# chto/linna

Hardware: AMD Instinct MI355X
Metric: emulator log-likelihood evals/sec (higher is better)
Workload: dtype f32; 1 GPU; 33-D Gaussian, 4x512 MLP emulator (33->512x4->33), nwalkers=4096 batched log-likelihood per GPU (BASELINE configs[1]); nwalkers_per_gpu=4096, launch=direct launches, parallelism=walkers sharded, 1 rank(s), no data-path collective

## Files before the change

include/linna_hip.h:

```cpp
#ifndef LINNA_HIP_H
#define LINNA_HIP_H
#include <stddef.h>
#include <stdint.h>

#ifdef __cplusplus
extern "C" {
#endif

#define LINNA_ABI_VERSION 12

typedef struct linna_ctx linna_ctx_t;
typedef struct linna_net linna_net_t;
typedef struct linna_logprob linna_logprob_t;
typedef struct linna_graph linna_graph_t;

int linna_abi_version(void);
const char* linna_last_error(void);
#define LINNA_OK 0
#define LINNA_ERR_INVALID (-1)
#define LINNA_ERR_HIP (-2)
#define LINNA_ERR_UNSUPPORTED (-3)
#define LINNA_ERR_INTERNAL (-4)
int linna_debug_raise(int kind);
int linna_ctx_create(int device, linna_ctx_t** out);
// ... 118 lines not shown
    const int* log10_flag; const float* xmean; const float* xstd;
    linna_colmap_t outmap;
    const float* S; int lds;
    const float* Ssym;
    const float* w;
    const float* gscale;
    float temperature;
    const float* Sfac;
} linna_logprob_desc_t;

int linna_logprob_create(linna_ctx_t* ctx, linna_net_t* net, const linna_logprob_desc_t* desc,
                         linna_logprob_t** out);
int linna_logprob_destroy(linna_logprob_t* lp);
int linna_weights_changed(linna_ctx_t* ctx);
#define LINNA_PRECISION_FP32 0
#define LINNA_PRECISION_BF16 1
int linna_logprob_set_precision(linna_logprob_t* lp, int precision);
int linna_logprob_precision(const linna_logprob_t* lp, int* out);
int linna_logprob_set_grad_precision(linna_logprob_t* lp, int precision);
int linna_logprob_grad_precision(const linna_logprob_t* lp, int* out);
int linna_engine_rows(int rows);
int linna_dense_tri(int mode);
int linna_serve_plain(int on);
int linna_program_plain(const linna_layer_t* layers, int nlayers, int in_size, int rows, int dense_nout);
int linna_logprob_serve_plain(linna_logprob_t* lp, int B, int* out);
int linna_logprob_grad_launches(linna_logprob_t* lp, int B, int* out);
int linna_slice_fusion(int mask);
int linna_program_describe(const linna_layer_t* layers, int nlayers, int in_size, int rows, int dense_nout, char* buf,
                           size_t n);
int linna_program_describe_grad_bf16(const linna_layer_t* layers, int nlayers, int in_size, int rows, char* buf, size_t n);
size_t linna_logprob_ws_bytes(const linna_logprob_t* lp, int B, int with_grad);
int linna_logprob_eval(linna_logprob_t* lp, const float* Z, int ldz, int B, void* ws, float* lnP,
                       float* THETA, int ldt, void* stream);
int linna_logprob_eval_if(linna_logprob_t* lp, const float* Z, int ldz, int B, void* ws, float* lnP,
                          float* THETA, int ldt, const int* gate, void* stream);
int linna_logprob_eval_slice_points(linna_logprob_t* lp, const float* coords, int ldc, int ndim, const int* S_idx,
                                    int ns, const float* DIR, int ldd, const float* w, int nrep, float* lnP,
                                    const int* gate, void* stream);
int linna_logprob_grad(linna_logprob_t* lp, const float* Z, int ldz, int B, void* ws, float* lnP,
                       float* G, int ldg, void* stream);
int linna_logprob_grad_leapfrog(linna_logprob_t* lp, float* Q, int ldq, int B, void* ws, float* lnP, float* G, int ldg,
                                float* P, int ldp, const float* mass, float eps_kick, float eps_drift, void* stream);

typedef struct {
    uint32_t struct_size;
    int nout;
// ... 165 lines not shown
```

linna_amd/_lib.py:

```python
import ctypes as C
import os

import torch

_HERE = os.path.dirname(os.path.abspath(__file__))
LIB_PATH = os.environ.get("LINNA_LIB_PATH") or os.path.join(_HERE, "liblinna_hip.so")
ABI_VERSION = 12

c_float_p = C.c_void_p
c_int_p = C.c_void_p


class _Sized(C.Structure):

    def __init__(self, *a, **k):
        C.Structure.__init__(self, *a, **k)
        self.struct_size = C.sizeof(type(self))


def sized_array(cls, n):
    arr = (cls * n)()
    for i in range(n):
        arr[i].struct_size = C.sizeof(cls)
    return arr
# ... 82 lines not shown
    "linna_linear_bwd": (_I, [_V, _V, _I, _V, _I, _V, _I, _V, _I, _V, _I, _V, _I, _V, _I, _I, _I, _F, _V]),
    "linna_net_create": (_I, [_V, C.POINTER(Layer), _I, _I, _PV]),
    "linna_net_destroy": (_I, [_V]),
    "linna_net_prepare": (_I, [_V, _I, _I]),
    "linna_net_fwd_ws_bytes": (_SZ, [_V, _I]),
    "linna_net_bwd_ws_bytes": (_SZ, [_V, _I]),
    "linna_net_forward": (_I, [_V, _V, _I, _I, _V, _V, _I, C.POINTER(ColMap), _V]),
    "linna_net_backward": (_I, [_V, _V, _I, _I, _V, _V, _V, _I, _V, _I, _I, _V]),
    "linna_net_stream_state": (_I, [_V, _V, _V, _V]),
    "linna_prior_map_fwd": (_I, [_V, _V, _I, _I, _I, _V, _V, _V, _V, _V, _V, _V, _I, _V, _I, _V]),
    "linna_prior_map_bwd": (_I, [_V, _V, _I, _I, _I, _V, _V, _V, _V, _V, _V, _I, _V, _I, _V]),
    "linna_gauss_loglike_diag": (_I, [_V, _V, _I, _I, _I, _V, _V, _I, _I, _F, _V, _V]),
    "linna_gauss_loglike_dense": (_I, [_V, _V, _I, _I, _I, _V, _I, _V, _I, _I, _F, _V, _V, _V]),
    "linna_logprob_create": (_I, [_V, _V, C.POINTER(LogprobDesc), _PV]),
    "linna_logprob_destroy": (_I, [_V]),
    "linna_weights_changed": (_I, [_V]),
    "linna_logprob_set_precision": (_I, [_V, _I]),
    "linna_logprob_precision": (_I, [_V, _V]),
    "linna_logprob_set_grad_precision": (_I, [_V, _I]),
    "linna_logprob_grad_precision": (_I, [_V, _V]),
    "linna_engine_rows": (_I, [_I]),
    "linna_dense_tri": (_I, [_I]),
    "linna_serve_plain": (_I, [_I]),
    "linna_program_plain": (_I, [_V, _I, _I, _I, _I]),
    "linna_logprob_serve_plain": (_I, [_V, _I, _V]),
    "linna_logprob_grad_launches": (_I, [_V, _I, _V]),
    "linna_slice_fusion": (_I, [_I]),
    "linna_net_train_launches": (_I, [_V, _I]),
    "linna_net_set_train_precision": (_I, [_V, _I]),
    "linna_net_train_precision": (_I, [_V, _V]),
    "linna_program_describe": (_I, [_V, _I, _I, _I, _I, _V, C.c_size_t]),
    "linna_program_describe_grad_bf16": (_I, [_V, _I, _I, _I, _V, C.c_size_t]),
    "linna_logprob_ws_bytes": (_SZ, [_V, _I, _I]),
    "linna_logprob_eval": (_I, [_V, _V, _I, _I, _V, _V, _V, _I, _V]),
    "linna_logprob_grad": (_I, [_V, _V, _I, _I, _V, _V, _V, _I, _V]),
    "linna_logprob_grad_leapfrog": (_I, [_V, _V, _I, _I, _V, _V, _V, _I, _V, _I, _V, _F, _F, _V]),
    "linna_loss_scratch_bytes": (_SZ, [_I, _I]),
    "linna_chi2_md": (_I, [_V, C.POINTER(LossDesc), _V, _I, _I, _V, _V, _V]),
    "linna_chi2_ratio_loss_fwd_bwd": (_I, [_V, C.POINTER(LossDesc), _V, _I, _V, _I, _V, _V, _I, _V, _V, _V, _V, _I, _F, _V]),
    "linna_net_prepare_loss": (_I, [_V, C.POINTER(LossDesc)]),
    "linna_loss_targets": (_I, [_V, C.POINTER(LossDesc), _V, _I, _I, _V, _I, _V]),
    "linna_net_forward_loss": (_I, [_V, C.POINTER(LossDesc), _V, _I, _V, _I, _V, _V, _V, _V, _I, _V, _V, _I, _V, _I, _V, _F, _V, _V, _V, _I,
                                    _V, _V, _F, _F, _V]),
    "linna_net_train_step": (_I, [_V, C.POINTER(LossDesc), _V, _I, _V, _I, _V, _V, _V, _V, _I, _V, _V, _I, _V, _I, _V, _F, _V, _V, _V, _I,
                                  _V, _V, _V, _F, _F, _V]),
    "linna_net_train_step_update": (_I, [_V, C.POINTER(LossDesc), _V, _I, _V, _I, _V, _V, _V, _V, _I, _V, _V, _I, _V, _I, _V, _F, _V, _V, _V, _I,
# ... 168 lines not shown
class quiet_gc(object):

    def __enter__(self):
        import gc
        self.on = gc.isenabled() and os.environ.get("LINNA_QUIET_GC", "1") != "0"
        if self.on:
            gc.freeze()
        return self

    def __exit__(self, *exc):
        import gc
        if self.on:
            gc.unfreeze()
        return False


def slice_fusion(mask=-1):
    prev = load().linna_slice_fusion(int(mask))
    if prev < 0:
        check(prev)
    return prev


def serve_plain(on=-1):
    prev = load().linna_serve_plain(int(on))
    if prev < 0:
        check(prev)
    return prev


def engine_rows(rows=0):
    prev = load().linna_engine_rows(int(rows))
    if prev < 0:
        check(prev)
    return prev
```

linna_amd/csrc/api.hip:

```cpp
#include "common.h"

#include <stdarg.h>
#include <stdio.h>
#include <string.h>
#include <cstring>
#include <string>
#include <vector>
#include <atomic>
#include <new>
#include <stdlib.h>

namespace linna {

static thread_local std::string g_err;

void set_error(const char* fmt, ...) {
    char buf[512];
    va_list ap;
    va_start(ap, fmt);
    vsnprintf(buf, sizeof buf, fmt, ap);
    va_end(ap);
    g_err = buf;
}

// ... 1029 lines not shown
    if (!lp || !out) { set_error("logprob_grad_precision: null argument"); return LINNA_ERR_INVALID; }
    *out = lp->grad_precision;
    return LINNA_OK;
} LINNA_CATCH_INT
int linna_program_describe_grad_bf16(const linna_layer_t* layers, int nlayers, int in_size, int rows, char* buf, size_t n) try {
    if (!layers || nlayers < 1 || !buf || !n) { set_error("program_describe_grad_bf16: bad arguments"); return LINNA_ERR_INVALID; }
    TRY(check_layers(layers, nlayers, "program_describe_grad_bf16"));
    return net_stream_describe(NS_GRAD_INPUT_BF16, layers, nlayers, in_size, nullptr, rows, buf, n);
} LINNA_CATCH_INT
int linna_program_describe(const linna_layer_t* layers, int nlayers, int in_size, int rows, int dense_nout, char* buf, size_t n) try {
    if (!layers || nlayers < 1 || !buf || !n) { set_error("program_describe: bad arguments"); return LINNA_ERR_INVALID; }
    TRY(check_layers(layers, nlayers, "program_describe"));
    static float dummy;
    if (dense_nout == -1) return net_stream_describe(ns_grad_kind(layers, nlayers), layers, nlayers, in_size, nullptr, rows, buf, n);
    const int dn_cols = dense_nout < -1 ? -dense_nout : dense_nout;
    NsDense dn{&dummy, (dn_cols + 3) & ~3, nullptr, nullptr, dense_nout < -1 ? 1 : 0, net_stream_dense_tri(-1)};
    if (dn_cols > 0) return net_stream_describe(NS_SERVE_DENSE, layers, nlayers, in_size, &dn, rows, buf, n);
    return net_stream_describe(NS_SERVE, layers, nlayers, in_size, nullptr, rows, buf, n);
} LINNA_CATCH_INT
int linna_serve_plain(int on) try {
    if (on < -1 || on > 1) { set_error("linna_serve_plain: %d (-1 query, 0 or 1)", on); return LINNA_ERR_INVALID; }
    return net_stream_serve_plain(on);
} LINNA_CATCH_INT
int linna_program_plain(const linna_layer_t* layers, int nlayers, int in_size, int rows, int dense_nout) try {
    if (!layers || nlayers < 1) { set_error("program_plain: bad arguments"); return LINNA_ERR_INVALID; }
    TRY(check_layers(layers, nlayers, "program_plain"));
    if (dense_nout != 0) return 0;
    return net_stream_program_plain(NS_SERVE, layers, nlayers, in_size, nullptr, rows) ? 1 : 0;
} LINNA_CATCH_INT
int linna_logprob_serve_plain(linna_logprob_t* lp, int B, int* out) try {
    if (!lp || !out || B < 1) { set_error("logprob_serve_plain: bad arguments"); return LINNA_ERR_INVALID; }
    static float dummy[4];
    const LpRun r = lp_fused_run(lp, LpRun{dummy, 0, B, dummy}, dummy, LpLayout{});
    const NsDense dn = lp->dense();
    *out = !lp->bf16() && lp_serves_fused(lp, false) && !lp->dense_fused &&
           net_stream_takes_plain(lp->kind(), net_layers(lp->net, lp->kind()), lp_output(lp), r.lnP, r.D, r.TH, nullptr, nullptr, r.gate,
                                  net_stream_rows(B), lp->kind() == NS_SERVE_DENSE ? &dn : nullptr);
    return LINNA_OK;
} LINNA_CATCH_INT
int linna_dense_tri(int mode) try {
    if (mode < -1 || mode > 2) { set_error("linna_dense_tri: %d (-1 query, 0, 1 or 2)", mode); return LINNA_ERR_INVALID; }
    return net_stream_dense_tri(mode);
} LINNA_CATCH_INT
static std::atomic<int> g_slice_fusion{7};
static bool slice_derive_enabled() { return (g_slice_fusion.load() & 1) != 0; }
int linna_slice_fusion(int mode) try {
// ... 699 lines not shown
```

linna_amd/csrc/common.h:

```cpp
#pragma once
#include <hip/hip_runtime.h>
#include <stdint.h>
#include <exception>
#include "../../include/linna_hip.h"


typedef float f32x4 __attribute__((ext_vector_type(4)));
typedef float f32x16 __attribute__((ext_vector_type(16)));

namespace linna {

struct U4 { uint32_t x, y, z, w; };
__device__ __forceinline__ U4 philox4x32_10(U4 c, uint32_t k0, uint32_t k1) {
#pragma unroll
    for (int r = 0; r < 10; ++r) {
        const uint64_t p0 = (uint64_t)0xD2511F53u * c.x;
        const uint64_t p1 = (uint64_t)0xCD9E8D57u * c.z;
        U4 n;
        n.x = (uint32_t)(p1 >> 32) ^ c.y ^ k0;
        n.y = (uint32_t)p1;
        n.z = (uint32_t)(p0 >> 32) ^ c.w ^ k1;
        n.w = (uint32_t)p0;
        c = n;
        k0 += 0x9E3779B9u; k1 += 0xBB67AE85u;
// ... 265 lines not shown
    NS_SERVE_DENSE,
    NS_SERVE_BF16,
    NS_STORE,
    NS_TRAIN_FWD,
    NS_DX,
    NS_DX_INPUT,
    NS_GRAD_INPUT,
    NS_TRAIN_STEP,
    NS_TRAIN_STEP_BF16,
    NS_GRAD_INPUT_BF16,
    NS_GRAD_INPUT_WIDE,
};
inline bool ns_kind_full_layers(NsKind k) { return k == NS_SERVE || k == NS_SERVE_DENSE || k == NS_SERVE_BF16; }
struct NsPlan { bool ok; size_t packed_floats; bool grad_ok; const char* why; };
NsPlan net_stream_plan(NsKind kind, const linna_layer_t* layers, int nl, int in_size, const NsDense* dn = nullptr);
int net_stream_rows(int B);
int net_stream_force_rows(int rows);
inline NsKind ns_grad_kind(const linna_layer_t* layers, int nl) { return nl >= 1 && layers[nl - 1].N > 64 ? NS_GRAD_INPUT_WIDE : NS_GRAD_INPUT; }
bool net_stream_grad_fits(const linna_layer_t* layers, int nl, int in_size, int rows);
int launch_net_stream_pack(NsKind kind, const linna_layer_t* layers, int nl, int in_size, float* packed, int rows, const NsDense* dn,
                           hipStream_t s);
int net_stream_describe(NsKind kind, const linna_layer_t* layers, int nl, int in_size, const NsDense* dn, int rows, char* buf, size_t n);
int net_stream_serve_plain(int on);
bool net_stream_program_plain(NsKind kind, const linna_layer_t* layers, int nl, int in_size, const NsDense* dn, int rows);
bool net_stream_launch_plain_ok(bool cscale, bool cshift, bool w, bool cexp, bool lnP, bool D, bool TH, bool gate);
struct NsNet { const linna_layer_t* layers; int nl, in_size; };
struct NsInput { int nin; const int* is_flat; const float* a1; const float* a2; const int* lg; const float* xmean; const float* xstd; };
struct NsOutput { const float* cscale; const float* cshift; const float* cpost; const float* cshift2; const float* w; float T; };
struct NsOpBufs { float* y; int ldy; float* t; int ldt; const float* x; int ldx; const float* gate; float* dprev; int ldp; float* dt; int lddt; };
struct NsPost { const float* rows; int n; float scale; float* out; int* step; float* hyper; float b1, b2; };
int launch_net_stream_dx(const NsNet& net, const float* packed, const float* dOUT, int lddo, int B, const NsOpBufs* ops, int with_input,
                         int rows, hipStream_t s, const NsPost* post = nullptr);
struct NsMove {
    float* coords; int ldc; float* logp; const int* S;
    const float* cc; int ldcc; const int* C; int nc;
    unsigned long long seed; const int* step; int step_off; int stream; float a; int* naccept;
    int slice;
    float* chain = nullptr; float* lps = nullptr;
    const float* sl_Z0 = nullptr; const float* sl_L = nullptr; const float* sl_R = nullptr; const float* sl_Zt = nullptr;
    int sl_m = 0, sl_nt = 0; unsigned long long sl_seed = 0; const int* sl_step = nullptr; int sl_stream = 0;
    const int* sl_flags = nullptr;
    const SliceBegin* sb = nullptr;
};
int launch_net_stream_store(const NsNet& net, const float* packed, const float* X, int ldx, int B, const NsOpBufs* ops,
                            const float* cscale, const float* cshift, int rows, hipStream_t s);
struct NsTrainLoss { const float* YN; int ldyn;
// ... 82 lines not shown
```

linna_amd/csrc/net_program.hip:

```cpp
#include "net_program.h"
#include <stdlib.h>
#include <algorithm>
#include <atomic>
#include <cstring>
#include <mutex>
#include <string>
#include <unordered_map>

namespace linna {

size_t NsProgram::lds_for(int rows, bool grad) const {
    size_t b = (size_t)(2 * rows * LD + ((bias_total + 3) & ~3)) * sizeof(float) + 128 + (x0_keep ? 4096 : 0);
#ifdef NS_STAMPS
    b += NS_NW * 32 * 8;
#endif
    return b + (grad ? (size_t)mask_slots * 64 * NS_NW * sizeof(unsigned) : 0);
}

static int ceil16(int k) { return (k + 15) & ~15; }
int ns_seg_steps(const NsSeg& s) {
    if (s.type == NS_WIDE && s.zext < 0) return 2 * s.steps - 60;
    return s.type == NS_WIDE && s.zext > 0 ? s.steps + (s.passes - 1) * s.zext : s.steps * s.passes;
}
static int ns_switch(std::atomic<int>& sw, const char* name, int dflt, bool (*valid)(int)) {
// ... 376 lines not shown
    if (cache.size() >= 256) cache.clear();
    NsProgramRef p = std::make_shared<const NsProgram>(ns_build_kind(kind, layers, nl, in_size, dn, side));
    cache.emplace(std::move(key), p);
    return p;
}

bool ns_program_plain(const NsProgram& p) {
    if (!p.ok || p.bf || p.dense || p.x0_keep || p.side_f4 || p.nseg_f < 1) return false;
    for (int i = 0; i < p.nseg_f; ++i) {
        const NsSeg& g = p.seg[i];
        if (g.type != NS_WIDE && g.type != NS_SPLIT) return false;
        if (g.x0_col || (g.type == NS_WIDE && (g.zext || g.kslice))) return false;
    }
    return true;
}
bool net_stream_program_plain(NsKind kind, const linna_layer_t* layers, int nl, int in_size, const NsDense* dn, int rows) {
    return kind == NS_SERVE && rows == 16 && ns_program_plain(*ns_program(kind, layers, nl, in_size, dn, rows));
}
bool net_stream_launch_plain_ok(bool cscale, bool cshift, bool w, bool cexp, bool lnP, bool D, bool TH, bool gate) {
    return cscale && cshift && w && !cexp && lnP && !D && !TH && !gate;
}
static std::atomic<int> g_serve_plain{1};
int net_stream_serve_plain(int on) { return on < 0 ? g_serve_plain.load() : g_serve_plain.exchange(on ? 1 : 0); }

int ns_seg_cols(const NsProgram& p, const linna_layer_t* layers, int i) {
    const linna_layer_t& l = layers[p.seg_op[i]];
    return p.seg_hidden[i] ? l.C : i < p.nseg_f ? l.N : l.K;
}
NsGates ns_gates(const NsProgram& p, const linna_layer_t* layers, int nl, int rows) {
    NsGates g;
    for (int i = 0; i < NS_MAXSEG; ++i) g.gbit[i] = g.mbit[i] = -1;
    for (int i = 0; i < p.nseg_f; ++i) {
        const int op = p.seg_op[i];
        if (op >= nl || (!p.seg_hidden[i] && op == nl - 1)) continue;
        g.gbit[i] = g.ncols;
        g.ncols += (ns_seg_cols(p, layers, i) + 63) & ~63;
    }
    for (int i = p.nseg_f; i < (int)p.seg.size(); ++i) {
        const int op = p.seg_op[i];
        const bool hidden = p.seg_hidden[i] != 0;
        if (!hidden && !(op > 0 && (layers[op - 1].op == LINNA_OP_RESBLOCK || layers[op - 1].relu))) continue;
        const int src = hidden ? op : op - 1;
        for (int j = 0; j < p.nseg_f; ++j)
            if (p.seg_op[j] == src && (p.seg_hidden[j] != 0) == hidden) g.mbit[i] = g.gbit[j];
        if (g.mbit[i] < 0) g.ok = false;
    }
// ... 188 lines not shown
```

linna_amd/csrc/net_stream.hip:

```cpp
#include "net_program.h"
#include <stdlib.h>
#include <type_traits>
#include <cstring>
#include <algorithm>

namespace linna {

typedef __bf16 bf16x8 __attribute__((ext_vector_type(8)));
typedef short s16x4 __attribute__((ext_vector_type(4)));

#ifndef NS_R
#define NS_R 6
#endif
#ifndef NS_PRE
#define NS_PRE 2
#endif
struct NsArgs {
    const float* Z; int ldz; int B; int nin;
    const int* is_flat; const float* a1; const float* a2; const int* lg;
    const float* xmean; const float* xstd;
    const float* packed;
    int G, nseg, LD, kpad0, nout, bias_total;
    int Gstride, nseg_f;
    const float* gscale; float* Gout; int ldg;
// ... 159 lines not shown
template <int R, int MOVE, bool GRAD, int STORE, int ROWS, bool BF = false>
__global__ __launch_bounds__(64 * NS_NW, 1) void net_stream_kernel(NsArgs a) {
    constexpr bool EPS = false, PLAIN = false, WOUT = false;
#include "net_stream_body.inc"
}
template <int R, int MOVE, bool GRAD, int STORE, int ROWS, bool BF>
__global__ __launch_bounds__(64 * NS_NW, 1) void net_stream_eps_kernel(NsArgs a) {
    static_assert(!BF && GRAD && (STORE == 0 || STORE == 2) && MOVE == 0, "the fp32 one-launch gradients only");
    constexpr bool EPS = true, PLAIN = false, WOUT = false;
#include "net_stream_body.inc"
}
template <int R, int MOVE, bool GRAD, int STORE, int ROWS, bool BF, bool EPSV>
__global__ __launch_bounds__(64 * NS_NW, 1) void net_stream_wide_kernel(NsArgs a) {
    static_assert(!BF && GRAD && STORE == 2 && MOVE == 0, "the fp32 one-launch gradient of any network only");
    constexpr bool EPS = EPSV, PLAIN = false, WOUT = true;
#include "net_stream_body.inc"
}
template <int R>
__global__ __launch_bounds__(64 * NS_NW, 1) void net_stream_plain_kernel(NsArgs a) {
    constexpr int MOVE = 0, STORE = 0, ROWS = 16;
    constexpr bool GRAD = false, BF = false, EPS = false, PLAIN = true, WOUT = false;
#include "net_stream_body.inc"
}
template <int R, int MOVE, bool GRAD, int STORE, int ROWS, bool BF>
__global__ __launch_bounds__(64 * NS_NW, 1) void net_stream_train_bf16_kernel(NsArgs a) {
    static_assert(BF && GRAD && STORE == 3 && ROWS == 4 && MOVE == 0, "the bf16 training step only");
    constexpr bool EPS = false, PLAIN = false, WOUT = false;
#include "net_stream_body.inc"
}
template <int R, int MOVE, bool GRAD, int STORE, int ROWS, bool BF>
__global__ __launch_bounds__(64 * NS_NW, 1) void net_stream_slice_bf16_kernel(NsArgs a) {
    static_assert(BF && !GRAD && STORE == 0 && MOVE == 2, "the bf16 slice evaluation only");
    constexpr bool EPS = false, PLAIN = false, WOUT = false;
#define NS_BODY_SLICE_BF16
#include "net_stream_body.inc"
#undef NS_BODY_SLICE_BF16
}
template <int R, int MOVE, bool GRAD, int STORE, int ROWS, bool BF>
__global__ __launch_bounds__(64 * NS_NW, 1) void net_stream_grad_bf16_kernel(NsArgs a) {
    static_assert(BF && GRAD && STORE == 2 && MOVE == 0, "the bf16 one-launch gradient only");
    constexpr bool EPS = false, PLAIN = false, WOUT = false;
#define NS_BODY_GRAD_BF16
#include "net_stream_body.inc"
#undef NS_BODY_GRAD_BF16
}
template <int R, int MOVE, bool GRAD, int STORE, int ROWS, bool BF>
// ... 57 lines not shown
        if (rc != LINNA_OK) return rc;
        attr_set = true;
    }
    hipLaunchKernelGGL(Kernel, dim3(nblocks), dim3(64 * NS_NW), lds_bytes, s, a);
    return check_hip(hipGetLastError(), what);
}
template <int MOVE, bool GRAD, int STORE, int ROWS, bool BF = false, bool EPS = false>
static int ns_launch_rows(const NsArgs& a, int B, size_t lds_bytes, hipStream_t s, int extra = 0) {
    if constexpr (EPS) return ns_launch<net_stream_eps_kernel<NS_R, MOVE, GRAD, STORE, ROWS, BF>>(a, (B + ROWS - 1) / ROWS + extra, lds_bytes, s, "net_stream launch");
    else return ns_launch<net_stream_kernel<NS_R, MOVE, GRAD, STORE, ROWS, BF>>(a, (B + ROWS - 1) / ROWS + extra, lds_bytes, s, "net_stream launch");
}
template <int MOVE, bool GRAD, int STORE = 0, bool BF = false, bool EPS = false>
static int ns_launch_kernel(const NsArgs& a0, int B, const NsProgram& p, int rows, hipStream_t s, int extra = 0, size_t lds_extra = 0,
                            bool plain = false, bool wide = false) {
    const size_t lds = p.lds_for(rows, GRAD) + lds_extra;
#ifdef NS_STAMPS
    NsArgs a = a0;
    a.stamps = getenv("LINNA_FUSED_STAMPS") ? reinterpret_cast<unsigned long long*>(strtoull(getenv("LINNA_FUSED_STAMPS"), nullptr, 16)) : nullptr;
    if (!a.stamps) { set_error("net_stream: NS_STAMPS build needs LINNA_FUSED_STAMPS"); return LINNA_ERR_INVALID; }
#else
    const NsArgs& a = a0;
#endif
    if constexpr (MOVE == 0 && !GRAD && STORE == 0 && !BF && !EPS) {
        if (plain && rows == 16) return ns_launch<net_stream_plain_kernel<NS_R>>(a, (B + 15) / 16, lds, s, "net_stream plain launch");
    }
    if constexpr (MOVE == 0 && GRAD && STORE == 2 && !BF) {
        const char* const what = "net_stream wide-output gradient launch";
        if (wide && rows == 4) return ns_launch<net_stream_wide_kernel<NS_R, 0, true, 2, 4, false, EPS>>(a, (B + 3) / 4, lds, s, what);
        if (wide && rows == 8) return ns_launch<net_stream_wide_kernel<NS_R, 0, true, 2, 8, false, EPS>>(a, (B + 7) / 8, lds, s, what);
        if (wide && rows == 16) return ns_launch<net_stream_wide_kernel<NS_R, 0, true, 2, 16, false, EPS>>(a, (B + 15) / 16, lds, s, what);
    }
    if (rows == 4) return ns_launch_rows<MOVE, GRAD, STORE, 4, BF, EPS>(a, B, lds, s, extra);
    if constexpr (BF) {
        if (rows == 8) return ns_launch_rows<MOVE, GRAD, STORE, 8, BF, EPS>(a, B, lds, s, extra);
        if (rows == 16) return ns_launch_rows<MOVE, GRAD, STORE, 16, BF, EPS>(a, B, lds, s, extra);
    } else if constexpr (STORE == 3 && GRAD) {
    } else {
        if (rows == 8) return ns_launch_rows<MOVE, GRAD, STORE, 8, false, EPS>(a, B, lds, s, extra);
        if (rows == 16) return ns_launch_rows<MOVE, GRAD, STORE, 16, false, EPS>(a, B, lds, s, extra);
    }
    set_error("net_stream: %d rows per workgroup", rows);
    return LINNA_ERR_INVALID;
}
template <int ROWS>
static int ns_launch_slice_bf16_rows(const NsArgs& a, int B, size_t lds_bytes, hipStream_t s) {
    return ns_launch<net_stream_slice_bf16_kernel<NS_R, 2, false, 0, ROWS, true>>(a, (B + ROWS - 1) / ROWS, lds_bytes, s, "net_stream bf16 slice launch");
// ... 331 lines not shown
```

linna_amd/csrc/net_stream_body.inc:

```
    constexpr int NT = NS_NT, NW = NS_NW;
    constexpr int RG = 32;
    constexpr bool SM = ROWS < 16;
    constexpr int RS = SM ? ROWS / 4 : 1;
    constexpr int NQ = SM ? RS : NT;
    constexpr int NACC = SM ? 4 * RS : NT;
#ifdef NS_BODY_SLICE_BF16
    static_assert(BF && !GRAD && STORE == 0 && MOVE == 2, "bf16: the slice evaluation");
#elif defined(NS_BODY_GRAD_BF16)
    static_assert(BF && GRAD && STORE == 2 && MOVE == 0, "bf16: lnP and its gradient in one launch");
#else
    static_assert(!BF || (!GRAD && STORE == 0 && MOVE != 2) || (GRAD && STORE == 3 && MOVE == 0 && ROWS == 4),
                  "bf16: serving, the fused stretch move and the merged training step (4-row engine)");
#endif
    constexpr bool BFT = BF && GRAD && STORE == 3;
    constexpr int AK = BF ? 2 : 1;
    constexpr bool K4 = !SM && !BF && (STORE == 0 || (GRAD && STORE == 2));
    constexpr bool TRB = GRAD && STORE == 3;
    constexpr bool DXE = STORE == 2 || TRB;
    constexpr bool G2 = GRAD && STORE == 2;
    constexpr bool LB = G2;
    constexpr bool LATE_REFILL = true;
    constexpr bool RNAN = STORE == 1;
    auto relu_f = [](float v) { if constexpr (RNAN) return isnan(v) ? v : fmaxf(v, 0.f); else return fmaxf(v, 0.f); };
    static_assert(ROWS == 16 || ROWS == 8 || ROWS == 4, "rows per workgroup");
    static_assert(R % 2 == 0, "the A double buffer alternates with the ring slot parity");
    extern __shared__ __attribute__((aligned(16))) float smem[];
    const int LD = a.LD, ABUF = ROWS * LD;
    constexpr bool KA = STORE == 3 || STORE == 1 || GRAD;
    const NsArgs* const ka = KA ? reinterpret_cast<const NsArgs*>((const void*)__builtin_amdgcn_kernarg_segment_ptr()) : &a;
    float* const act = smem;
    float* const lbias = smem + 2 * ABUF;
    unsigned* const lbits = reinterpret_cast<unsigned*>(smem + a.bits_off);
    const int nbw = a.nbw;
    const int tid = threadIdx.x, lane = tid & 63;
    const int wave = __builtin_amdgcn_readfirstlane(tid >> 6);
    const int li = lane & 15, kq = lane >> 4;
    const int row0 = blockIdx.x * ROWS;
    if constexpr (!PLAIN) {
        if (a.gate && a.gate[0] == 0) return;
    }
    int mv_rows = a.B;
    if constexpr (MOVE == 2) {
        if (a.mv_C) {
            mv_rows = a.mv_step[0] * a.mv_step_off;
// ... 310 lines not shown
        if (j < nb4) reinterpret_cast<f32x4*>(lbias)[j] = breg[i];
    }
    int* const lsrc = reinterpret_cast<int*>(lbias + ((a.bias_total + 3) & ~3));
    float* const lden = reinterpret_cast<float*>(lsrc + 16);
    if constexpr (STORE == 3) {
        if (prow && pc0 == 0) { lsrc[pr] = zsrc; lden[pr] = zden; }
    }
    float* const lx0 = lden + 16;
    if constexpr (!PLAIN) {
    if (a.x0_keep && prow) {
#pragma unroll
        for (int i = 0; i < ZPRE; ++i) {
            const int c = pc0 + i * RG;
            if constexpr (BF) lx0[pr * 64 + c] = c < nin ? act[pr * LD + c] + act[pr * LD + nin + c] : 0.f;
            else lx0[pr * 64 + c] = (c < kpad0) ? act[pr * LD + c] : 0.f;
        }
    }
    }
    asm volatile("s_waitcnt lgkmcnt(0)" ::: "memory");
    __builtin_amdgcn_s_barrier();
    asm volatile("" ::: "memory");
    NS_STAMP();

    const uint32_t act_lds = (uint32_t)(uintptr_t)(__attribute__((address_space(3))) void*)act;
    f32x4 acc[NACC];
    f32x4 Aq[2][AK];
    const int sm_arow = (4 * ((lane >> 2) & 3) + (lane & 3)) % ROWS, sm_achunk = lane >> 4;
    int si = 0, pass = 0, P = 0, kleft;
    int s_type, s_steps, s_passes, s_bias, s_dst, s_relu, s_kslice, s_zext, s_ncgl, s_mstore = 0, s_mapply = 0, s_x0col = 0, s_x0n = 0, s_kcl = 0;
    unsigned* const lmask = reinterpret_cast<unsigned*>(lbias + ((a.bias_total + 3) & ~3));
    float lnp_grad = 0.f;
    float* s_gout = nullptr; int s_gld = 0, s_gn = 0;
    const float* s_gmask = nullptr; int s_gmld = 0;
    int s_gbit = -1, s_mbit = -1;
    auto gstore = [&](float* p, float v) { asm volatile("global_store_dword %0, %1, off" :: "v"(p), "v"(v) : "memory"); };
    uint32_t ap;
    auto a_read = [&](f32x4* dst) {
        asm volatile("ds_read_b128 %0, %1" : "=v"(dst[0]) : "v"(ap) : "memory");
        if constexpr (BF) asm volatile("ds_read_b128 %0, %1 offset:16" : "=v"(dst[1]) : "v"(ap) : "memory");
        if constexpr (BFT) ap += si == a.nseg_f - 1 ? 64 : 64 * AK;
        else ap += 64 * AK;
    };
    auto load_seg = [&]() {
        const NsSeg S = ka->seg[__builtin_amdgcn_readfirstlane(si)];
        s_type = S.type; kleft = s_steps = S.steps; s_passes = S.passes; s_bias = S.bias_off;
        s_dst = S.dst_col; s_relu = S.relu; s_kslice = S.kslice; s_zext = S.zext; s_ncgl = S.ncg_log2; s_x0col = S.x0_col; s_x0n = S.x0_n;
        if constexpr (GRAD) { s_mstore = S.mask_store; s_mapply = S.mask_apply; }
        if constexpr (STORE) { const int j = __builtin_amdgcn_readfirstlane(si); s_gout = ka->gout[j]; s_gld = ka->gld[j]; s_gn = ka->gn[j]; }
        if constexpr (DXE) { const int j = __builtin_amdgcn_readfirstlane(si); s_gmask = ka->gmask[j]; s_gmld = ka->gmld[j]; }
        if constexpr (LB) { const int j = __builtin_amdgcn_readfirstlane(si); s_gbit = ka->gbit[j]; s_mbit = ka->mbit[j]; }
    };
    NsSeg nxp;
    auto plain_request = [&]() { nxp = ka->seg[__builtin_amdgcn_readfirstlane(min(si + 1, nseg - 1))]; };
    auto plain_take = [&](const NsSeg& X) {
        s_type = X.type & 255; s_ncgl = X.type >> 8; kleft = s_steps = X.steps; s_passes = X.passes; s_bias = X.bias_off;
        s_dst = X.dst_col; s_relu = X.relu; s_kslice = X.kslice; s_zext = X.zext;
    };
    auto begin_run = [&]() {
        const int arow = SM ? sm_arow : li, ak = AK * (SM ? 4 * sm_achunk : 4 * kq);
#pragma unroll
        for (int t = 0; t < NACC; ++t) acc[t] = f32x4{0.f, 0.f, 0.f, 0.f};
        if (s_type == NS_WIDE) {
            const int blk = !PLAIN && s_zext < 0 ? (pass ? 15 - wave : wave) : 8 * pass + wave;
            if constexpr (SM) {
                const float b = lbias[s_bias + 64 * blk + lane];
#pragma unroll
                for (int r = 0; r < RS; ++r) acc[4 * r] = f32x4{b, b, b, b};
            } else {
#pragma unroll
                for (int t = 0; t < NT; ++t) {
                    const float b = lbias[s_bias + 16 * (4 * blk + t) + li];
                    acc[t] = f32x4{b, b, b, b};
                }
            }
            if (!PLAIN && s_zext < 0) kleft = s_steps - 4 * blk;
            ap = act_lds + 4u * (uint32_t)(P * ABUF + arow * LD + ak + (PLAIN ? 0 : s_zext < 0 ? 64 * blk : (pass ? s_kslice : 0)));
        } else {
            ap = act_lds + 4u * (uint32_t)(P * ABUF + arow * LD + ak + (wave >> s_ncgl) * s_kslice);
        }
        if constexpr (BFT) {
            if (si == a.nseg_f - 1) ap -= 4u * (uint32_t)(ak / 2);
        }
    };
    auto lds_barrier = [&]() {
        asm volatile("s_waitcnt lgkmcnt(0)" ::: "memory");
        __builtin_amdgcn_s_barrier();
        asm volatile("" ::: "memory");
    };
    if constexpr (PLAIN) {
        asm volatile("" :: "s"(seg_warm));
        plain_take(ka->seg[0]); begin_run(); a_read(Aq[0]); plain_request();
    }
    else {
    load_seg();
    begin_run();
    a_read(Aq[0]);
    }

    auto step = [&](auto Uc, auto Refill) {
        constexpr int U = decltype(Uc)::value;
        constexpr bool refill = decltype(Refill)::value;
        constexpr int RU = LATE_REFILL ? (U + R - 1) % R : U;
        if constexpr (BF) asm volatile("s_waitcnt lgkmcnt(0)" : "+v"(Aq[U & 1][0]), "+v"(Aq[U & 1][AK - 1]) :: "memory");
        else asm volatile("s_waitcnt lgkmcnt(0)" : "+v"(Aq[U & 1][0]) :: "memory");
        a_read(Aq[(U + 1) & 1]);
        const f32x4 av = Aq[U & 1][0];
        if constexpr (BF) {
            bf16x8 ab;
#pragma unroll
            for (int e = 0; e < 4; ++e) { ab[e] = (__bf16)Aq[U & 1][0][e]; ab[4 + e] = (__bf16)Aq[U & 1][AK - 1][e]; }
            if constexpr (SM) {
                auto bf_small = [&]() {
                    const s16x4 alo = __builtin_bit_cast(s16x4, __builtin_shufflevector(ab, ab, 0, 1, 2, 3));
                    const s16x4 ahi = __builtin_bit_cast(s16x4, __builtin_shufflevector(ab, ab, 4, 5, 6, 7));
#define NS_B4(r, c, h, A4) acc[4 * (r) + (c)] = __builtin_amdgcn_mfma_f32_4x4x4bf16_1k(A4, \
                __builtin_bit_cast(s16x4, __builtin_shufflevector(__builtin_bit_cast(bf16x8, Bq[U][c]), __builtin_bit_cast(bf16x8, Bq[U][c]), \
                                                                  4 * (h), 4 * (h) + 1, 4 * (h) + 2, 4 * (h) + 3)), acc[4 * (r) + (c)], 4, 4 * (c) + (r), 0);
#define NS_B4R(r, h, A4) NS_B4(r, 0, h, A4) NS_B4(r, 1, h, A4) NS_B4(r, 2, h, A4) NS_B4(r, 3, h, A4)
                    NS_B4R(0, 0, alo)
                    if constexpr (RS > 1) { NS_B4R(1, 0, alo) }
                    NS_B4R(0, 1, ahi)
                    if constexpr (RS > 1) { NS_B4R(1, 1, ahi) }
#undef NS_B4R
#undef NS_B4
                };
// ... 38 lines not shown
                if constexpr (RS > 1) { NS_M4R(1, e) }
            }
#undef NS_M4R
#undef NS_M4
            if constexpr (refill) {
#pragma unroll
                for (int t = 0; t < NT; ++t) Bq[RU][t] = wload(t);
            }
        } else {
#pragma unroll
            for (int h = 0; h < NT; h += 2) {
#pragma unroll
                for (int s = 0; s < 4; ++s) {
                    acc[h] = __builtin_amdgcn_mfma_f32_16x16x4f32(av[s], Bq[U][h][s], acc[h], 0, 0, 0);
                    acc[h + 1] = __builtin_amdgcn_mfma_f32_16x16x4f32(av[s], Bq[U][h + 1][s], acc[h + 1], 0, 0, 0);
                }
                if constexpr (refill) {
                    Bq[RU][h] = wload(h);
                    Bq[RU][h + 1] = wload(h + 1);
                }
            }
        }
        if constexpr (refill) wadvance();
        if (--kleft == 0) {
            const int nxi = __builtin_amdgcn_readfirstlane(min(si + 1, nseg - 1));
            const NsSeg NX = ka->seg[nxi];
            float* nx_gout = nullptr; int nx_gld = 0, nx_gn = 0;
            const float* nx_gmask = nullptr; int nx_gmld = 0;
            if constexpr (STORE) { nx_gout = ka->gout[nxi]; nx_gld = ka->gld[nxi]; nx_gn = ka->gn[nxi]; }
            if constexpr (DXE) { nx_gmask = ka->gmask[nxi]; nx_gmld = ka->gmld[nxi]; }
            int nx_gbit = -1, nx_mbit = -1;
            if constexpr (LB) { nx_gbit = ka->gbit[nxi]; nx_mbit = ka->mbit[nxi]; }
            const int cur_steps = s_steps;
            auto take_seg = [&](const NsSeg& X) {
                s_type = X.type; s_steps = X.steps; s_passes = X.passes; s_bias = X.bias_off;
                s_dst = X.dst_col; s_relu = X.relu; s_kslice = X.kslice; s_zext = X.zext; s_ncgl = X.ncg_log2; s_x0col = X.x0_col; s_x0n = X.x0_n;
                if constexpr (K4) s_kcl = X.kcl;
                if constexpr (GRAD) { s_mstore = X.mask_store; s_mapply = X.mask_apply; }
                kleft = X.steps;
            };
            auto take_next = [&]() {
                if constexpr (PLAIN) { plain_take(nxp); return; }
                take_seg(NX);
                if constexpr (STORE) { s_gout = nx_gout; s_gld = nx_gld; s_gn = nx_gn; }
                if constexpr (DXE) { s_gmask = nx_gmask; s_gmld = nx_gmld; }
                if constexpr (LB) { s_gbit = nx_gbit; s_mbit = nx_mbit; }
            };
// ... 616 lines not shown
                for (int j = 0; j < ZPRE; ++j)
                    if (pc0 + j * RG < nin) a.mv_coords[(size_t)mv_wk * a.mv_ldc + pc0 + j * RG] = zr[j];
                if (pc0 == 0) {
                    a.mv_logp[mv_wk] = lnp_new;
                    if (a.mv_naccept) a.mv_naccept[mv_wk] += 1;
                }
            }
            if (a.mv_chain && rok) {
#pragma unroll
                for (int j = 0; j < ZPRE; ++j)
                    if (pc0 + j * RG < nin)
                        a.mv_chain[(size_t)mv_wk * nin + pc0 + j * RG] = mv_acc ? zr[j] : a.mv_coords[(size_t)mv_wk * a.mv_ldc + pc0 + j * RG];
                if (pc0 == 0) a.mv_lps[mv_wk] = mv_acc ? lnp_new : mv_lnp_old;
            }
        }
        if (!PLAIN && a.TH && rok) {
#pragma unroll
            for (int j = 0; j < ZPRE; ++j)
                if (pc0 + j * RG < nin) a.TH[(size_t)(row0 + pr) * a.ldt + pc0 + j * RG] = theta[j];
            for (int c = pc0 + ZPRE * RG; c < nin; c += RG)
                a.TH[(size_t)(row0 + pr) * a.ldt + c] = ns_prior_theta(a.Z[(size_t)grow * a.ldz + c], a.is_flat[c], a.a1[c], a.a2[c]);
        }
    }
    NS_STAMP();
    NS_STAMPS_FLUSH();
#undef NS_STAMP
#undef NS_STAMPS_FLUSH
```

Measured before the change: 75.31 million evals/s.

## Add hand-scheduled inline-asm inner step for plain fp32 serving kernel

Adds a new kernel variant for plain fp32 serving with 16 rows and six weight slots. Its inner K-step is written as inline assembly with pinned VGPRs for the weight ring, activations and accumulators. The MFMA ops, LDS activation reads, global weight refills and waitcnt thresholds are interleaved by hand to hide load latency better than the compiler schedule. A runtime switch selects this path and defaults to on. The cost is fragile hardcoded register allocation and vmcnt counts, plus explicit nops for MFMA hazards.

```diff
diff --git a/include/linna_hip.h b/include/linna_hip.h
--- a/include/linna_hip.h
+++ b/include/linna_hip.h
@@ -164,6 +164,7 @@
 int linna_engine_rows(int rows);
 int linna_dense_tri(int mode);
 int linna_serve_plain(int on);
+int linna_serve_plain_sched(int hand);
 int linna_program_plain(const linna_layer_t* layers, int nlayers, int in_size, int rows, int dense_nout);
 int linna_logprob_serve_plain(linna_logprob_t* lp, int B, int* out);
 int linna_logprob_grad_launches(linna_logprob_t* lp, int B, int* out);
diff --git a/linna_amd/_lib.py b/linna_amd/_lib.py
--- a/linna_amd/_lib.py
+++ b/linna_amd/_lib.py
@@ -128,6 +128,7 @@
     "linna_engine_rows": (_I, [_I]),
     "linna_dense_tri": (_I, [_I]),
     "linna_serve_plain": (_I, [_I]),
+    "linna_serve_plain_sched": (_I, [_I]),
     "linna_program_plain": (_I, [_V, _I, _I, _I, _I]),
     "linna_logprob_serve_plain": (_I, [_V, _I, _V]),
     "linna_logprob_grad_launches": (_I, [_V, _I, _V]),
@@ -342,6 +343,13 @@
     return prev
 
 
+def serve_plain_sched(hand=-1):
+    prev = load().linna_serve_plain_sched(int(hand))
+    if prev < 0:
+        check(prev)
+    return prev
+
+
 def serve_plain(on=-1):
     prev = load().linna_serve_plain(int(on))
     if prev < 0:
diff --git a/linna_amd/csrc/api.hip b/linna_amd/csrc/api.hip
--- a/linna_amd/csrc/api.hip
+++ b/linna_amd/csrc/api.hip
@@ -1075,6 +1075,10 @@
     if (on < -1 || on > 1) { set_error("linna_serve_plain: %d (-1 query, 0 or 1)", on); return LINNA_ERR_INVALID; }
     return net_stream_serve_plain(on);
 } LINNA_CATCH_INT
+int linna_serve_plain_sched(int hand) try {
+    if (hand < -1 || hand > 1) { set_error("linna_serve_plain_sched: %d (-1 query, 0 or 1)", hand); return LINNA_ERR_INVALID; }
+    return net_stream_serve_plain_sched(hand);
+} LINNA_CATCH_INT
 int linna_program_plain(const linna_layer_t* layers, int nlayers, int in_size, int rows, int dense_nout) try {
     if (!layers || nlayers < 1) { set_error("program_plain: bad arguments"); return LINNA_ERR_INVALID; }
     TRY(check_layers(layers, nlayers, "program_plain"));
diff --git a/linna_amd/csrc/common.h b/linna_amd/csrc/common.h
--- a/linna_amd/csrc/common.h
+++ b/linna_amd/csrc/common.h
@@ -311,6 +311,7 @@
                            hipStream_t s);
 int net_stream_describe(NsKind kind, const linna_layer_t* layers, int nl, int in_size, const NsDense* dn, int rows, char* buf, size_t n);
 int net_stream_serve_plain(int on);
+int net_stream_serve_plain_sched(int hand);
 bool net_stream_program_plain(NsKind kind, const linna_layer_t* layers, int nl, int in_size, const NsDense* dn, int rows);
 bool net_stream_launch_plain_ok(bool cscale, bool cshift, bool w, bool cexp, bool lnP, bool D, bool TH, bool gate);
 struct NsNet { const linna_layer_t* layers; int nl, in_size; };
diff --git a/linna_amd/csrc/net_program.hip b/linna_amd/csrc/net_program.hip
--- a/linna_amd/csrc/net_program.hip
+++ b/linna_amd/csrc/net_program.hip
@@ -422,6 +422,8 @@
 }
 static std::atomic<int> g_serve_plain{1};
 int net_stream_serve_plain(int on) { return on < 0 ? g_serve_plain.load() : g_serve_plain.exchange(on ? 1 : 0); }
+static std::atomic<int> g_serve_plain_sched{1};
+int net_stream_serve_plain_sched(int hand) { return hand < 0 ? g_serve_plain_sched.load() : g_serve_plain_sched.exchange(hand ? 1 : 0); }
 
 int ns_seg_cols(const NsProgram& p, const linna_layer_t* layers, int i) {
     const linna_layer_t& l = layers[p.seg_op[i]];
diff --git a/linna_amd/csrc/net_stream.hip b/linna_amd/csrc/net_stream.hip
--- a/linna_amd/csrc/net_stream.hip
+++ b/linna_amd/csrc/net_stream.hip
@@ -205,6 +205,17 @@
     constexpr bool GRAD = false, BF = false, EPS = false, PLAIN = true, WOUT = false;
 #include "net_stream_body.inc"
 }
+#if NS_R == 6
+#define NS_HAVE_PLACED 1
+template <int R>
+__global__ __launch_bounds__(64 * NS_NW, 1) void net_stream_placed_kernel(NsArgs a) {
+    constexpr int MOVE = 0, STORE = 0, ROWS = 16;
+    constexpr bool GRAD = false, BF = false, EPS = false, PLAIN = true, WOUT = false;
+#define NS_BODY_HAND
+#include "net_stream_body.inc"
+#undef NS_BODY_HAND
+}
+#endif
 template <int R, int MOVE, bool GRAD, int STORE, int ROWS, bool BF>
 __global__ __launch_bounds__(64 * NS_NW, 1) void net_stream_train_bf16_kernel(NsArgs a) {
     static_assert(BF && GRAD && STORE == 3 && ROWS == 4 && MOVE == 0, "the bf16 training step only");
@@ -308,6 +319,10 @@
     const NsArgs& a = a0;
 #endif
     if constexpr (MOVE == 0 && !GRAD && STORE == 0 && !BF && !EPS) {
+#ifdef NS_HAVE_PLACED
+        if (plain && rows == 16 && net_stream_serve_plain_sched(-1))
+            return ns_launch<net_stream_placed_kernel<NS_R>>(a, (B + 15) / 16, lds, s, "net_stream plain launch (hand-placed step)");
+#endif
         if (plain && rows == 16) return ns_launch<net_stream_plain_kernel<NS_R>>(a, (B + 15) / 16, lds, s, "net_stream plain launch");
     }
     if constexpr (MOVE == 0 && GRAD && STORE == 2 && !BF) {
diff --git a/linna_amd/csrc/net_stream_body.inc b/linna_amd/csrc/net_stream_body.inc
--- a/linna_amd/csrc/net_stream_body.inc
+++ b/linna_amd/csrc/net_stream_body.inc
@@ -20,6 +20,21 @@
     constexpr bool G2 = GRAD && STORE == 2;
     constexpr bool LB = G2;
     constexpr bool LATE_REFILL = true;
+#ifdef NS_BODY_HAND
+    constexpr bool HAND = true;
+    static_assert(PLAIN && !BF && ROWS == 16 && R == 6 && NS_NT == 4 && LATE_REFILL, "the hand-placed step: plain fp32 serving, 16 rows, six slots");
+#else
+    constexpr bool HAND = false;
+#endif
+#define NS_HAND_RING \
+    "+{v[128:131]}"(Bq[0][0]), "+{v[132:135]}"(Bq[0][1]), "+{v[136:139]}"(Bq[0][2]), "+{v[140:143]}"(Bq[0][3]), \
+    "+{v[144:147]}"(Bq[1][0]), "+{v[148:151]}"(Bq[1][1]), "+{v[152:155]}"(Bq[1][2]), "+{v[156:159]}"(Bq[1][3]), \
+    "+{v[160:163]}"(Bq[2][0]), "+{v[164:167]}"(Bq[2][1]), "+{v[168:171]}"(Bq[2][2]), "+{v[172:175]}"(Bq[2][3]), \
+    "+{v[176:179]}"(Bq[3][0]), "+{v[180:183]}"(Bq[3][1]), "+{v[184:187]}"(Bq[3][2]), "+{v[188:191]}"(Bq[3][3]), \
+    "+{v[192:195]}"(Bq[4][0]), "+{v[196:199]}"(Bq[4][1]), "+{v[200:203]}"(Bq[4][2]), "+{v[204:207]}"(Bq[4][3]), \
+    "+{v[208:211]}"(Bq[5][0]), "+{v[212:215]}"(Bq[5][1]), "+{v[216:219]}"(Bq[5][2]), "+{v[220:223]}"(Bq[5][3])
+#define NS_HAND_A "+{v[224:227]}"(Aq[0][0]), "+{v[228:231]}"(Aq[1][0])
+#define NS_HAND_ACC "+{v[232:235]}"(acc[0]), "+{v[236:239]}"(acc[1]), "+{v[240:243]}"(acc[2]), "+{v[244:247]}"(acc[3])
     constexpr bool RNAN = STORE == 1;
     auto relu_f = [](float v) { if constexpr (RNAN) return isnan(v) ? v : fmaxf(v, 0.f); else return fmaxf(v, 0.f); };
     static_assert(ROWS == 16 || ROWS == 8 || ROWS == 4, "rows per workgroup");
@@ -376,6 +391,11 @@
     asm volatile("" ::: "memory");
     NS_STAMP();
 
+    if constexpr (HAND) {
+#pragma unroll
+        for (int t = 0; t < NT; ++t) Bq[R - 1][t] = f32x4{0.f, 0.f, 0.f, 0.f};
+        asm volatile("" : NS_HAND_RING :: "memory");
+    }
     const uint32_t act_lds = (uint32_t)(uintptr_t)(__attribute__((address_space(3))) void*)act;
     f32x4 acc[NACC];
     f32x4 Aq[2][AK];
@@ -390,6 +410,10 @@
     auto gstore = [&](float* p, float v) { asm volatile("global_store_dword %0, %1, off" :: "v"(p), "v"(v) : "memory"); };
     uint32_t ap;
     auto a_read = [&](f32x4* dst) {
+        if constexpr (HAND) {
+            if (dst == Aq[0]) asm volatile("ds_read_b128 %0, %1" : "={v[224:227]}"(Aq[0][0]) : "v"(ap) : "memory");
+            else asm volatile("ds_read_b128 %0, %1" : "={v[228:231]}"(Aq[1][0]) : "v"(ap) : "memory");
+        } else
         asm volatile("ds_read_b128 %0, %1" : "=v"(dst[0]) : "v"(ap) : "memory");
         if constexpr (BF) asm volatile("ds_read_b128 %0, %1 offset:16" : "=v"(dst[1]) : "v"(ap) : "memory");
         if constexpr (BFT) ap += si == a.nseg_f - 1 ? 64 : 64 * AK;
@@ -435,6 +459,7 @@
         if constexpr (BFT) {
             if (si == a.nseg_f - 1) ap -= 4u * (uint32_t)(ak / 2);
         }
+        if constexpr (HAND) asm volatile("s_nop 3" : NS_HAND_ACC);
     };
     auto lds_barrier = [&]() {
         asm volatile("s_waitcnt lgkmcnt(0)" ::: "memory");
@@ -455,6 +480,58 @@
         constexpr int U = decltype(Uc)::value;
         constexpr bool refill = decltype(Refill)::value;
         constexpr int RU = LATE_REFILL ? (U + R - 1) % R : U;
+        if constexpr (HAND) {
+            constexpr int BU = 128 + 16 * U, BR = 128 + 16 * RU, AC = 224 + 4 * (U & 1), AN = 224 + 4 * ((U + 1) & 1);
+            constexpr int TW = refill ? 0 : 4 * U;
+#define NS_HM(t, s) "v_mfma_f32_16x16x4_f32 v[232+4*" #t ":235+4*" #t "], v[%[ac]+" #s "], v[%[bu]+4*" #t "+" #s "], v[232+4*" #t ":235+4*" #t "]\n\t"
+#define NS_HL(t, off) "global_load_dwordx4 v[%[ru]+4*" #t ":%[ru]+4*" #t "+3], %[vo], %[sb] offset:" #off "\n\t"
+#define NS_HAND_TEXT(HEAD, L0, L1, L2, L3) HEAD \
+            "s_waitcnt lgkmcnt(0)\n\t" \
+            "s_waitcnt vmcnt(%[w0])\n\t" \
+            NS_HM(0, 0) "ds_read_b128 v[%[an]:%[an]+3], %[ap]\n\t" \
+            "s_waitcnt vmcnt(%[w1])\n\t" \
+            NS_HM(1, 0) \
+            NS_HM(0, 1) L0 \
+            NS_HM(1, 1) \
+            NS_HM(0, 2) L1 \
+            NS_HM(1, 2) \
+            NS_HM(0, 3) L2 \
+            NS_HM(1, 3) \
+            "s_waitcnt vmcnt(%[w2])\n\t" \
+            NS_HM(2, 0) L3 \
+            "s_waitcnt vmcnt(%[w3])\n\t" \
+            NS_HM(3, 0) \
+            NS_HM(2, 1) "v_add_u32 %[ap], 64, %[ap]\n\t" \
+            NS_HM(3, 1) NS_HM(2, 2) NS_HM(3, 2) NS_HM(2, 3) NS_HM(3, 3)
+            if constexpr (refill) {
+                const char* const sb = wbase + woff;
+#ifdef NS_HAND_PHASE4
+#define NS_HAND_HEAD ".p2align 3\n\ts_nop 0\n\t"
+#else
+#define NS_HAND_HEAD ".p2align 3\n\t"
+#endif
+                if constexpr (U == 0)
+                    asm volatile(NS_HAND_TEXT(NS_HAND_HEAD, NS_HL(0, 0), NS_HL(1, 1024), NS_HL(2, 2048), NS_HL(3, 3072))
+                                 : NS_HAND_RING, NS_HAND_A, NS_HAND_ACC, [ap] "+v"(ap)
+                                 : [vo] "v"(voff), [sb] "s"(sb), [bu] "n"(BU), [ru] "n"(BR), [ac] "n"(AC), [an] "n"(AN),
+                                   [w0] "n"(19), [w1] "n"(18), [w2] "n"(20), [w3] "n"(20) : "memory");
+                else
+                    asm volatile(NS_HAND_TEXT("", NS_HL(0, 0), NS_HL(1, 1024), NS_HL(2, 2048), NS_HL(3, 3072))
+                                 : NS_HAND_RING, NS_HAND_A, NS_HAND_ACC, [ap] "+v"(ap)
+                                 : [vo] "v"(voff), [sb] "s"(sb), [bu] "n"(BU), [ru] "n"(BR), [ac] "n"(AC), [an] "n"(AN),
+                                   [w0] "n"(19), [w1] "n"(18), [w2] "n"(20), [w3] "n"(20) : "memory");
+                wadvance();
+            } else {
+                asm volatile(NS_HAND_TEXT("", "", "", "", "")
+                             : NS_HAND_RING, NS_HAND_A, NS_HAND_ACC, [ap] "+v"(ap)
+                             : [bu] "n"(BU), [ac] "n"(AC), [an] "n"(AN),
+                               [w0] "n"(19 - TW), [w1] "n"(18 - TW), [w2] "n"(17 - TW), [w3] "n"(16 - TW) : "memory");
+            }
+#undef NS_HAND_TEXT
+#undef NS_HAND_HEAD
+#undef NS_HL
+#undef NS_HM
+        } else {
         if constexpr (BF) asm volatile("s_waitcnt lgkmcnt(0)" : "+v"(Aq[U & 1][0]), "+v"(Aq[U & 1][AK - 1]) :: "memory");
         else asm volatile("s_waitcnt lgkmcnt(0)" : "+v"(Aq[U & 1][0]) :: "memory");
         a_read(Aq[(U + 1) & 1]);
@@ -539,7 +616,9 @@
             }
         }
         if constexpr (refill) wadvance();
+        }
         if (--kleft == 0) {
+            if constexpr (HAND) asm volatile("s_nop 15" : NS_HAND_ACC);
             const int nxi = __builtin_amdgcn_readfirstlane(min(si + 1, nseg - 1));
             const NsSeg NX = ka->seg[nxi];
             float* nx_gout = nullptr; int nx_gld = 0, nx_gn = 0;
@@ -1202,7 +1281,11 @@
                 a.TH[(size_t)(row0 + pr) * a.ldt + c] = ns_prior_theta(a.Z[(size_t)grow * a.ldz + c], a.is_flat[c], a.a1[c], a.a2[c]);
         }
     }
+    if constexpr (HAND) asm volatile("" : NS_HAND_RING);
     NS_STAMP();
     NS_STAMPS_FLUSH();
 #undef NS_STAMP
 #undef NS_STAMPS_FLUSH
+#undef NS_HAND_RING
+#undef NS_HAND_A
+#undef NS_HAND_ACC
```

After: 76.39 million evals/s (median of 6 runs). 1.01x the previous value.
